# PKBeam/Lanczos-HLS

Hardware: AMD Instinct MI355X
Metric: output Mpixels/s (higher is better)
Workload: dtype f32; 1 GPU; 1920x1080->3840x2160 RGB8 2x Lanczos-3; batch_sets_cycled=3, pattern=gradient, parity_mode=lsb1, kernel=fast, parallelism=32 frames per GPU per step over 1 GPU(s), no data-path collective

## Files before the change

### lanczos-hls_amd/csrc/lanczos_api.hip

```cpp
#include <hip/hip_runtime.h>

#include <algorithm>
#include <cstdio>
#include <cstdlib>
#include <cstring>
#include <map>
#include <mutex>
#include <new>
#include <vector>

#include "../../include/lanczos_hip.h"
#include "lanczos_env.hpp"
#include "lanczos_fast.hpp"
#include "lanczos_layout.hpp"
#include "lanczos_march.hpp"
#include "lanczos_generic.hpp"
#include "lanczos_hls.hpp"
#include "lanczos_rational.hpp"
#include "lanczos_resize.hpp"
#include "lanczos_kernels_common.hpp"
#include "lanczos_taps.hpp"

namespace {

struct PlanKey {
    int in_w, in_h, out_w, out_h, channels, bps, sn, sd, a, hls;
    bool operator<(const PlanKey& o) const { return memcmp(this, &o, sizeof(PlanKey)) < 0; }
};

struct Plan {
    PlanKey key;
    std::vector<hipStream_t> streams;
    lz::AxisTaps H, V;
    lz::PrefixInfo prefix;
    lz::TapTables dev{};
    void* dev_block = nullptr;
    void* host_block = nullptr;
    hipEvent_t uploaded = nullptr;
    hipStream_t upload_stream = nullptr;
    bool captured = false;
    lz::FastConsts fast{};
    bool fast_ok = false;
    lz::RatHost rat;
    lz::RatTables rat_dev{};
    lz::RatPHost ratp;
    lz::RatTables ratp_dev{};
    const float* ratp_w_dev = nullptr;
};

}

struct lanczos_ctx {
    int device = 0;
    hipStream_t stream = nullptr;
    std::map<PlanKey, Plan*> plans;
    lz::LruOrder<PlanKey> plan_order;
    lz::RetireList retired_plans;
    std::vector<void*> kept_dev, kept_host;
    std::mutex mu;
    int last_kernel = LANCZOS_KERNEL_NONE;
    int last_tensor_route = 0;
    int last_route = 0;
    int route_launches = 0;
    int route_seen = 0;
    int last_hip = 0;
    int force = LANCZOS_KERNEL_NONE;
    void* stage_in = nullptr;
    void* stage_out = nullptr;
    size_t stage_in_bytes = 0, stage_out_bytes = 0;
    bool timing = false;
    std::vector<hipEvent_t> ev;
    std::vector<char> ev_prefix_first;
    int ev_used = 0;
    int launches = 0;
    double main_ms = 0, prefix_ms = 0;
#ifdef LZ_PROFILE_BITS
    void* stamp_buf = nullptr;
#endif
    lz::WgTabCache wg_tabs;
    hipStream_t copy_in = nullptr, copy_out = nullptr;
    std::vector<hipEvent_t> pipe_ev;
    void* planar_in = nullptr;
    void* planar_out = nullptr;
    size_t planar_in_bytes = 0, planar_out_bytes = 0;
    lz::ResizeState* resize = nullptr;
};
#ifdef LZ_PROFILE_BITS
static constexpr size_t kStampBytes = 16384 * 8 * 6 * 8;
#endif
static constexpr size_t kMaxPlans = 32;
#ifndef LZ_SPLIT_RULE
#define LZ_SPLIT_RULE 1
#endif

namespace {

#define LZ_HIP(ctx, call)                                  \
    do {                                                   \
        hipError_t e_ = (call);                            \
        if (e_ != hipSuccess) {                            \
            (ctx)->last_hip = (int)e_;                     \
            return LANCZOS_ERR_HIP;                        \
        }                                                  \
    } while (0)

void route_begin(lanczos_ctx* ctx) { ctx->last_route = ctx->route_launches = ctx->route_seen = ctx->last_tensor_route = 0; }
void route_launch(lanczos_ctx* ctx, int main_kernel, int prefix_route) {
    if (ctx->route_launches < 0x7fff) ctx->route_launches++;
    ctx->route_seen |= 1 << prefix_route;
    ctx->last_route = main_kernel | prefix_route << 4 | ctx->route_seen << 8 | ctx->route_launches << 16;
}

void free_plan(Plan* p) {
    if (p->dev_block) (void)hipFree(p->dev_block);
    if (p->host_block) (void)hipHostFree(p->host_block);
    if (p->uploaded) (void)hipEventDestroy(p->uploaded);
    delete p;
}

int get_plan(lanczos_ctx* ctx, const lanczos_desc* d, hipStream_t stream, Plan** out) {
    PlanKey key;
    memset(&key, 0, sizeof(key));
    const bool hls = d->mode == LANCZOS_MODE_HLS;
    key = PlanKey{d->in_w, d->in_h, d->out_w, d->out_h, d->channels, d->bytes_per_sample,
                  d->scale_n, d->scale_d, d->a, hls ? 1 + d->reserved[0] : 0};
    auto it = ctx->plans.find(key);
    if (it != ctx->plans.end()) {
        Plan* p = it->second;
        ctx->plan_order.touch(key);
        if (lz::stream_capturing(stream)) {
            if (p->uploaded && hipEventQuery(p->uploaded) != hipSuccess) LZ_HIP(ctx, hipEventSynchronize(p->uploaded));
            p->captured = true;
        } else {
            if (p->uploaded && stream != p->upload_stream && hipEventQuery(p->uploaded) != hipSuccess)
                LZ_HIP(ctx, hipStreamWaitEvent(stream, p->uploaded, 0));
            lz::note_stream(p->streams, stream);
        }
        *out = p;
        return LANCZOS_OK;
    }
    ctx->retired_plans.reap(false);
    if (ctx->plans.size() >= kMaxPlans && !ctx->plan_order.empty()) {
        const PlanKey old = ctx->plan_order.pop_oldest();
        auto io = ctx->plans.find(old);
        if (io != ctx->plans.end()) {
            Plan* q = io->second;
            if (q->captured) {
                ctx->kept_dev.push_back(q->dev_block);
                ctx->kept_host.push_back(q->host_block);
            } else {
                ctx->retired_plans.retire({q->dev_block}, {q->host_block}, q->streams);
            }
            if (q->uploaded) (void)hipEventDestroy(q->uploaded);
            delete q;
            ctx->plans.erase(io);
        }
    }
    Plan* p = new (std::nothrow) Plan();
    if (!p) return LANCZOS_ERR_NOMEM;
    p->key = key;
    if (hls) {
        lz::build_axis_hls(d->in_w, d->out_w, d->scale_n, d->scale_d, d->a, &p->H, d->reserved[0]);
        lz::build_axis_hls(d->in_h, d->out_h, d->scale_n, d->scale_d, d->a, &p->V, d->reserved[0]);
    } else {
        lz::build_axis(d->in_w, d->out_w, d->scale_n, d->scale_d, d->a, &p->H);
        lz::build_axis(d->in_h, d->out_h, d->scale_n, d->scale_d, d->a, &p->V);
        p->prefix = lz::prefix_info(p->V);
    }
    const int taps = 2 * d->a;
    size_t off_hf = 0;
    size_t off_vf = off_hf + (((size_t)d->out_w * 4 + 7) & ~(size_t)7);
    size_t off_hw = off_vf + (((size_t)d->out_h * 4 + 7) & ~(size_t)7);
    size_t off_vw = off_hw + (size_t)d->out_w * taps * 8;
    size_t off_xw = off_vw + (size_t)d->out_h * taps * 8;
    size_t total = off_xw + (size_t)lz::kFastMaxS * lz::kMaxTaps * 8;
    p->fast_ok = !hls && lz::fast_prepare(*d, p->H, p->V, &p->fast);
    if (!hls && d->scale_d != 1) lz::rat_prepare(*d, p->H, p->V, &p->rat);
    size_t off_hwf = 0, off_vwf = 0, off_hint = 0, off_vint = 0;
    if (p->rat.ok) {
        off_hwf = total;
        off_vwf = off_hwf + (size_t)d->out_w * taps * 4;
        off_hint = off_vwf + (size_t)d->out_h * taps * 4;
        off_vint = off_hint + (((size_t)d->out_w + 7) & ~(size_t)7);
        total = off_vint + (((size_t)d->out_h + 7) & ~(size_t)7);
    }
    size_t off_pw = 0;
    if (p->rat.ok && lz::ratp_has(*d)) lz::ratp_prepare(*d, p->H, p->V, p->rat, &p->ratp);
    if (p->ratp.ok) {
        off_pw = total;
        total += sizeof(p->ratp.phase_w);
    }
    hipError_t e = hipHostMalloc(&p->host_block, total, hipHostMallocDefault);
    if (e != hipSuccess) {
        ctx->last_hip = (int)e;
        delete p;
        return LANCZOS_ERR_HIP;
    }
    struct HostView {
        uint8_t* b;
        uint8_t* data() const { return b; }
    } host{(uint8_t*)p->host_block};
    memset(host.data(), 0, total);
    if (p->rat.ok) {
        memcpy(host.data() + off_hwf, p->rat.h_wf.data(), p->rat.h_wf.size() * 4);
        memcpy(host.data() + off_vwf, p->rat.v_wf.data(), p->rat.v_wf.size() * 4);
        memcpy(host.data() + off_hint, p->rat.h_int.data(), p->rat.h_int.size());
        memcpy(host.data() + off_vint, p->rat.v_int.data(), p->rat.v_int.size());
    }
    if (p->ratp.ok) memcpy(host.data() + off_pw, p->ratp.phase_w, sizeof(p->ratp.phase_w));
    if (p->fast_ok) {
        memcpy(host.data() + off_xw, p->fast.wi, lz::kMaxTaps * 8);
        for (int ph = 1; ph < lz::kFastMaxS; ph++)
            memcpy(host.data() + off_xw + (size_t)ph * lz::kMaxTaps * 8, p->fast.wd[ph], lz::kMaxTaps * 8);
    }
    memcpy(host.data() + off_hf, p->H.first.data(), (size_t)d->out_w * 4);
    memcpy(host.data() + off_vf, p->V.first.data(), (size_t)d->out_h * 4);
    memcpy(host.data() + off_hw, p->H.w.data(), (size_t)d->out_w * taps * 8);
    memcpy(host.data() + off_vw, p->V.w.data(), (size_t)d->out_h * taps * 8);
    const bool capturing = lz::stream_capturing(stream);
    hipStream_t up = stream;
    e = hipMalloc(&p->dev_block, total);
    if (e == hipSuccess && capturing) e = ctx->wg_tabs.eager_stream(&up);
    if (e == hipSuccess && !capturing) e = hipEventCreateWithFlags(&p->uploaded, hipEventDisableTiming);
    if (e != hipSuccess) {
        ctx->last_hip = (int)e;
        free_plan(p);
        return LANCZOS_ERR_HIP;
    }
    e = hipMemcpyAsync(p->dev_block, p->host_block, total, hipMemcpyHostToDevice, up);
    if (e == hipSuccess) e = capturing ? hipStreamSynchronize(up) : hipEventRecord(p->uploaded, stream);
    if (e != hipSuccess) {
        ctx->last_hip = (int)e;
        ctx->retired_plans.retire({p->dev_block}, {p->host_block}, {up});
        if (p->uploaded) (void)hipEventDestroy(p->uploaded);
        delete p;
        return LANCZOS_ERR_HIP;
    }
    if (capturing) {
        p->captured = true;
    } else {
        p->upload_stream = stream;
        p->streams.push_back(stream);
    }
    uint8_t* b = (uint8_t*)p->dev_block;
    p->dev.h_first = (const int32_t*)(b + off_hf);
    p->dev.v_first = (const int32_t*)(b + off_vf);
    p->dev.h_w = (const double*)(b + off_hw);
    p->dev.v_w = (const double*)(b + off_vw);
    p->dev.x_w = (const double*)(b + off_xw);
    if (p->rat.ok) {
        p->rat_dev.h_wf = (const float*)(b + off_hwf);
        p->rat_dev.v_wf = (const float*)(b + off_vwf);
        p->rat_dev.h_int = b + off_hint;
        p->rat_dev.v_int = b + off_vint;
        p->rat_dev.bias = p->rat.bias;
        p->rat_dev.vbias_rne = p->rat.vbias_rne;
        p->rat_dev.near2 = p->rat.near2;
        p->rat_dev.vlim = p->rat.vlim;
        p->rat_dev.tight = p->rat.tight;
    }
    if (p->ratp.ok) {
        p->ratp_dev = p->rat_dev;
        p->ratp_dev.bias = p->ratp.bias;
        p->ratp_dev.vbias_rne = p->ratp.vbias_rne;
        p->ratp_dev.near2 = p->ratp.near2;
        p->ratp_w_dev = (const float*)(b + off_pw);
    }
    ctx->plans[key] = p;
    ctx->plan_order.touch(key);
    *out = p;
    return LANCZOS_OK;
}

int whole_or_strip(const lanczos_desc* d, int* row0, int* rows) {
    if (d->out_rows == 0) {
        *row0 = 0;
        *rows = d->out_h;
    } else {
        *row0 = d->out_row0;
        *rows = d->out_rows;
    }
    return LANCZOS_OK;
}

void strip_input_rows(const lz::AxisTaps& V, int a, int in_h, int row0, int rows, const lz::PrefixInfo& pi,
                      int* in_row0, int* in_rows) {
    int lo = V.first[row0];
    int hi = V.first[row0 + rows - 1] + 2 * a - 1;
    if (row0 < pi.K && pi.M2 - 1 > hi) hi = pi.M2 - 1;
    if (lo < 0) lo = 0;
    if (hi > in_h - 1) hi = in_h - 1;
    *in_row0 = lo;
    *in_rows = hi - lo + 1;
}

}

extern "C" {

const char* lanczos_version(void) {
#ifdef LZ_PROFILE_BITS
    return "lanczos-hls_amd 0.1 (gfx950) +profile-bits";
#else
    return "lanczos-hls_amd 0.1 (gfx950)";
#endif
}

const char* lanczos_strerror(int code) {
    switch (code) {
        case LANCZOS_OK: return "ok";
        case LANCZOS_ERR_BAD_ARG: return "bad argument (null pointer, size, channels, a, or out != in*N/D)";
        case LANCZOS_ERR_UNSUPPORTED: return "unsupported configuration (scale < 1, or a strip that cuts the in-place prefix rows)";
        case LANCZOS_ERR_NO_DEVICE: return "no HIP device";
        case LANCZOS_ERR_HIP: return "HIP runtime error";
        case LANCZOS_ERR_NOMEM: return "out of memory";
        case LANCZOS_ERR_RCCL: return "RCCL call failed (lanczos_multi_last_error)";
        default: return "unknown error";
    }
}

int lanczos_desc_init(lanczos_desc* d, int in_w, int in_h, int channels, int bytes_per_sample, int scale_n,
                      int scale_d, int a) {
    if (!d) return LANCZOS_ERR_BAD_ARG;
    memset(d, 0, sizeof(*d));
    if (scale_n <= 0 || scale_d <= 0) return LANCZOS_ERR_BAD_ARG;
    const int g = lz::gcd(scale_n, scale_d);
    d->in_w = in_w;
    d->in_h = in_h;
    d->scale_n = scale_n / g;
    d->scale_d = scale_d / g;
    d->out_w = (int)((long long)in_w * d->scale_n / d->scale_d);
    d->out_h = (int)((long long)in_h * d->scale_n / d->scale_d);
    d->channels = channels;
    d->bytes_per_sample = bytes_per_sample;
    d->a = a;
    d->mode = LANCZOS_MODE_LSB1;
    return lz::validate(d);
}

int lanczos_validate(const lanczos_desc* d) { return lz::validate(d); }

int lanczos_inplace_rows(const lanczos_desc* d) {
    if (lz::validate(d) != LANCZOS_OK) return -1;
    if (d->mode == LANCZOS_MODE_HLS) return 0;
    lz::AxisTaps V;
    lz::build_axis(d->in_h, d->out_h, d->scale_n, d->scale_d, d->a, &V);
    return lz::prefix_info(V).K;
}

int lanczos_strip_input_rows(const lanczos_desc* d, int out_row0, int out_rows, int* in_row0, int* in_rows) {
    int rc = lz::validate(d);
    if (rc != LANCZOS_OK) return rc;
    if (!in_row0 || !in_rows || out_row0 < 0 || out_rows <= 0 || out_row0 + out_rows > d->out_h)
        return LANCZOS_ERR_BAD_ARG;
    lz::AxisTaps V;
    if (d->mode == LANCZOS_MODE_HLS) {
        lz::build_axis_hls(d->in_h, d->out_h, d->scale_n, d->scale_d, d->a, &V, d->reserved[0]);
        strip_input_rows(V, d->a, d->in_h, out_row0, out_rows, lz::PrefixInfo(), in_row0, in_rows);
        return LANCZOS_OK;
    }
    lz::build_axis(d->in_h, d->out_h, d->scale_n, d->scale_d, d->a, &V);
    strip_input_rows(V, d->a, d->in_h, out_row0, out_rows, lz::prefix_info(V), in_row0, in_rows);
    return LANCZOS_OK;
}

size_t lanczos_in_frame_bytes(const lanczos_desc* d) {
    return d ? (size_t)d->in_w * d->in_h * d->channels * d->bytes_per_sample : 0;
}
size_t lanczos_out_frame_bytes(const lanczos_desc* d) {
    return d ? (size_t)d->out_w * d->out_h * d->channels * d->bytes_per_sample : 0;
}

double lanczos_kernel(double x, int a) { return lz::kernel(x, a); }

double lanczos_kernel_idx(int in_idx, int out_idx, int scale_n, int scale_d, int a) {
    const double SCALE = (double)scale_n / scale_d;
    const double x = (double)out_idx / SCALE;
    return lz::kernel(x - in_idx, a);
}

int lanczos_taps_host(const lanczos_desc* d, int axis, int32_t* first, double* weights) {
    int rc = lz::validate(d);
    if (rc != LANCZOS_OK) return rc;
    if (!first || !weights || (axis != 0 && axis != 1)) return LANCZOS_ERR_BAD_ARG;
    lz::AxisTaps t;
    if (d->mode == LANCZOS_MODE_HLS)
        lz::build_axis_hls(axis == 0 ? d->in_w : d->in_h, axis == 0 ? d->out_w : d->out_h, d->scale_n, d->scale_d, d->a, &t, d->reserved[0]);
    else if (axis == 0)
        lz::build_axis(d->in_w, d->out_w, d->scale_n, d->scale_d, d->a, &t);
    else
        lz::build_axis(d->in_h, d->out_h, d->scale_n, d->scale_d, d->a, &t);
    memcpy(first, t.first.data(), t.first.size() * sizeof(int32_t));
    memcpy(weights, t.w.data(), t.w.size() * sizeof(double));
    return LANCZOS_OK;
}

int lanczos_create(lanczos_ctx** out, int device) {
    if (!out) return LANCZOS_ERR_BAD_ARG;
    *out = nullptr;
    int n = 0;
    if (hipGetDeviceCount(&n) != hipSuccess || n <= 0) return LANCZOS_ERR_NO_DEVICE;
    if (device < 0 || device >= n) return LANCZOS_ERR_NO_DEVICE;
    (void)lz::env();
    lanczos_ctx* ctx = new (std::nothrow) lanczos_ctx();
    if (!ctx) return LANCZOS_ERR_NOMEM;
    ctx->device = device;
    if (hipSetDevice(device) != hipSuccess ||
        hipStreamCreateWithFlags(&ctx->stream, hipStreamNonBlocking) != hipSuccess) {
        delete ctx;
        return LANCZOS_ERR_HIP;
    }
    *out = ctx;
    return LANCZOS_OK;
}

#ifdef LZ_PROFILE_BITS
static void diag_report(lanczos_ctx* ctx, FILE* out) {
    if (!ctx->stamp_buf) return;
    {
        std::vector<unsigned long long> h(kStampBytes / 8);
        if (hipMemcpy(h.data(), ctx->stamp_buf, kStampBytes, hipMemcpyDeviceToHost) == hipSuccess) {
            double sum[5] = {0, 0, 0, 0, 0}, ticks = 0;
            long n = 0;
            for (size_t i = 0; i + 5 < (size_t)16384 * 8 * 3; i += 6)
                if (h[i + 5]) {
                    for (int k = 0; k < 5; k++) sum[k] += (double)h[i + k];
                    ticks += (double)h[i + 5];
                    n++;
                }
            {
                std::map<unsigned long long, std::vector<std::pair<unsigned long long, int>>> ev;
                const size_t off = (size_t)16384 * 8 * 3;
                long wgs = 0;
                unsigned long long tmin = ~0ull, tmax = 0;
                for (size_t i = off; i + 2 < h.size(); i += 3) {
                    if (!h[i + 1]) continue;
                    const unsigned hw = (unsigned)h[i + 2];
                    const unsigned long long key = ((h[i + 2] >> 32) << 16) | (((hw >> 13) & 7) << 8) | (((hw >> 12) & 1) << 4) | ((hw >> 8) & 15);
                    ev[key].push_back({h[i], +1});
                    ev[key].push_back({h[i + 1], -1});
                    if (h[i] < tmin) tmin = h[i];
                    if (h[i + 1] > tmax) tmax = h[i + 1];
                    wgs++;
                }
                double avg = 0;
                int peak = 0;
                for (auto& kv : ev) {
                    std::sort(kv.second.begin(), kv.second.end());
                    int cur = 0;
                    unsigned long long last = tmin, area = 0;
                    for (auto& e : kv.second) {
                        area += (unsigned long long)cur * (e.first - last);
                        last = e.first;
                        cur += e.second;
                        if (cur > peak) peak = cur;
                    }
                    avg += (double)area / (double)(tmax - tmin ? tmax - tmin : 1);
                }
                {
                    std::vector<double> st, life;
                    for (size_t i = off; i + 2 < h.size(); i += 3)
                        if (h[i + 1]) {
                            st.push_back((h[i] - tmin) / 100.0);
                            life.push_back((h[i + 1] - h[i]) / 100.0);
                        }
                    std::sort(st.begin(), st.end());
                    std::sort(life.begin(), life.end());
                    if (!st.empty())
                        fprintf(out, "CENSUS start us: p50=%.1f p90=%.1f max=%.1f | lifetime us: min=%.1f p10=%.1f p50=%.1f p90=%.1f max=%.1f\n",
                                st[st.size() / 2], st[st.size() * 9 / 10], st.back(), life.front(), life[life.size() / 10],
                                life[life.size() / 2], life[life.size() * 9 / 10], life.back());
                }
                if (!lz::env().census_dump.empty()) {
                    FILE* df = fopen(lz::env().census_dump.c_str(), "w");
                    if (df) {
                        for (size_t i = off, k = 0; i + 2 < h.size(); i += 3, k++)
                            if (h[i + 1])
                                fprintf(df, "%zu %llu %llu %u %u\n", k, h[i] - tmin, h[i + 1] - tmin, (unsigned)(h[i + 2] >> 32),
                                        (unsigned)h[i + 2]);
                        fclose(df);
                    }
                }
                if (wgs)
                    fprintf(out, "CENSUS wgs=%ld distinct_cus=%zu span=%.1f us avg_resident_wgs_per_cu=%.2f peak=%d\n", wgs,
                            ev.size(), (tmax - tmin) / 100.0, avg / ev.size(), peak);
            }
            if (n)
                fprintf(out, "STAMP waves=%ld ticks/wave=%.1f cycles/tick: issue=%.0f hpass=%.0f commit=%.0f vpass=%.0f barrier=%.0f\n",
                        n, ticks / n, sum[0] / ticks, sum[1] / ticks, sum[2] / ticks, sum[3] / ticks, sum[4] / ticks);
            for (int w = 0; w < 6; w++) {
                double s6[5] = {0, 0, 0, 0, 0}, tk = 0;
                for (size_t i = (size_t)w * 6; i + 5 < (size_t)16384 * 8 * 3; i += 36)
                    if (h[i + 5]) {
                        for (int k = 0; k < 5; k++) s6[k] += (double)h[i + k];
                        tk += (double)h[i + 5];
                    }
                if (tk > 0)
                    fprintf(out, "STAMP wave %d: issue=%.0f hpass=%.0f commit=%.0f vpass=%.0f barrier=%.0f\n", w, s6[0] / tk, s6[1] / tk,
                            s6[2] / tk, s6[3] / tk, s6[4] / tk);
            }
        }
    }
}
#endif

int lanczos_destroy(lanczos_ctx* ctx) {
    if (!ctx) return LANCZOS_ERR_BAD_ARG;
    (void)hipSetDevice(ctx->device);
    (void)hipDeviceSynchronize();
    ctx->retired_plans.reap(true);
    ctx->wg_tabs.release_all();
    for (auto& kv : ctx->plans) free_plan(kv.second);
    ctx->plans.clear();
    for (void* p : ctx->kept_dev) (void)hipFree(p);
    for (void* p : ctx->kept_host) (void)hipHostFree(p);
    delete ctx->resize;
#ifdef LZ_PROFILE_BITS
    if (ctx->stamp_buf) {
        diag_report(ctx, stderr);
        (void)hipFree(ctx->stamp_buf);
    }
#endif
    for (hipEvent_t e : ctx->ev) (void)hipEventDestroy(e);
    for (hipEvent_t e : ctx->pipe_ev) (void)hipEventDestroy(e);
    if (ctx->copy_in) (void)hipStreamDestroy(ctx->copy_in);
    if (ctx->copy_out) (void)hipStreamDestroy(ctx->copy_out);
    if (ctx->planar_in) (void)hipFree(ctx->planar_in);
    if (ctx->planar_out) (void)hipFree(ctx->planar_out);
    if (ctx->stage_in) (void)hipFree(ctx->stage_in);
    if (ctx->stage_out) (void)hipFree(ctx->stage_out);
    if (ctx->stream) (void)hipStreamDestroy(ctx->stream);
    delete ctx;
    return LANCZOS_OK;
}

int lanczos_timing_enable(lanczos_ctx* ctx, int on) {
    if (!ctx) return LANCZOS_ERR_BAD_ARG;
    ctx->timing = on != 0;
    return LANCZOS_OK;
}

static int timing_flush(lanczos_ctx* ctx) {
    const int used = ctx->ev_used;
    ctx->ev_used = 0;
    for (int i = 0; i + 2 < used; i += 3) {
        float a = 0, b = 0;
        LZ_HIP(ctx, hipEventSynchronize(ctx->ev[i + 2]));
        LZ_HIP(ctx, hipEventElapsedTime(&a, ctx->ev[i], ctx->ev[i + 1]));
        LZ_HIP(ctx, hipEventElapsedTime(&b, ctx->ev[i + 1], ctx->ev[i + 2]));
        const bool prefix_first = ctx->ev_prefix_first[i / 3] != 0;
        ctx->main_ms += prefix_first ? b : a;
        ctx->prefix_ms += prefix_first ? a : b;
        ctx->launches++;
    }
    return LANCZOS_OK;
}

int lanczos_timing_read(lanczos_ctx* ctx, int* launches, double* main_kernel_ms, double* prefix_kernel_ms) {
    if (!ctx) return LANCZOS_ERR_BAD_ARG;
    std::lock_guard<std::mutex> lock(ctx->mu);
    (void)hipSetDevice(ctx->device);
    int rc = timing_flush(ctx);
    if (rc != LANCZOS_OK) return rc;
    if (launches) *launches = ctx->launches;
    if (main_kernel_ms) *main_kernel_ms = ctx->main_ms;
    if (prefix_kernel_ms) *prefix_kernel_ms = ctx->prefix_ms;
    ctx->launches = 0;
    ctx->main_ms = ctx->prefix_ms = 0;
    return LANCZOS_OK;
}

int lanczos_last_kernel(const lanczos_ctx* ctx) { return ctx ? ctx->last_kernel : LANCZOS_KERNEL_NONE; }
int lanczos_last_route(const lanczos_ctx* ctx) { return ctx ? ctx->last_route : 0; }
int lanczos_last_hip_error(const lanczos_ctx* ctx) { return ctx ? ctx->last_hip : 0; }

int lanczos_force_kernel(lanczos_ctx* ctx, int family) {
    if (!ctx || family < LANCZOS_KERNEL_NONE || family > LANCZOS_KERNEL_FAST) return LANCZOS_ERR_BAD_ARG;
    ctx->force = family;
    return LANCZOS_OK;
}

static hipError_t launch_prefix_front(const lanczos_desc* d, const lz::FrameGeom& g, const Plan* p, hipStream_t stream) {
#define LZ_PREFIX_REG_CONFIGS(X)                                                                                        \
    X(uint8_t, 2, 2) X(uint8_t, 2, 3) X(uint8_t, 2, 4) X(uint8_t, 3, 2) X(uint8_t, 3, 3) X(uint8_t, 3, 4) X(uint8_t, 4, 2) \
    X(uint8_t, 4, 3) X(uint8_t, 4, 4) X(uint16_t, 2, 3) X(uint16_t, 2, 4) X(uint16_t, 3, 3) X(uint16_t, 3, 4)
    bool have = false;
#define X(T, S, A)                                                                                                    \
    if (d->bytes_per_sample == (int)sizeof(T) && d->scale_n == S && d->a == A && p->prefix.K == lz::prefix_K(S, A) && \
        p->prefix.M == lz::prefix_M(S, A) && p->prefix.M2 == lz::prefix_M2(S, A))                                    \
        have = true;
    LZ_PREFIX_REG_CONFIGS(X)
#undef X
    if (!have) return hipErrorNotSupported;
    const int samples_w = d->out_w * d->channels;
    dim3 grid((samples_w + 127) / 128, g.frames);
#define X(T, S, A)                                                                                  \
    if (d->bytes_per_sample == (int)sizeof(T) && d->scale_n == S && d->a == A)                      \
        hipLaunchKernelGGL((lz::k_prefix_reg<T, S, A>), grid, dim3(128), 0, stream, g, p->dev);
    LZ_PREFIX_REG_CONFIGS(X)
#undef X
    return hipGetLastError();
}

static int resample_device_locked(lanczos_ctx* ctx, const lanczos_desc* d, const void* d_in, void* d_out, int frames,
                                  size_t in_frame_stride, size_t out_frame_stride, void* stream_v, bool in_split = false) {
    int rc;
    LZ_HIP(ctx, hipSetDevice(ctx->device));
    hipStream_t stream = (hipStream_t)stream_v;
    Plan* p = nullptr;
    rc = get_plan(ctx, d, stream, &p);
    if (rc != LANCZOS_OK) return rc;

    int row0, rows;
    whole_or_strip(d, &row0, &rows);
    int in_row0, in_rows;
    strip_input_rows(p->V, d->a, d->in_h, row0, rows, p->prefix, &in_row0, &in_rows);
    const bool has_prefix = row0 < p->prefix.K;
    if (has_prefix) {
        if (row0 != 0) return LANCZOS_ERR_UNSUPPORTED;
    }

    lz::FrameGeom g{};
    g.in = (const uint8_t*)d_in;
    g.out = (uint8_t*)d_out;
    g.in_pitch = d->in_w * d->channels * d->bytes_per_sample;
    g.out_pitch = d->out_w * d->channels * d->bytes_per_sample;
    g.in_frame_stride = in_frame_stride ? in_frame_stride : (size_t)g.in_pitch * in_rows;
    g.out_frame_stride = out_frame_stride ? out_frame_stride : (size_t)g.out_pitch * rows;
    g.in_w = d->in_w;
    g.in_h = d->in_h;
    g.out_w = d->out_w;
    g.out_h = d->out_h;
    g.channels = d->channels;
    g.a = d->a;
    g.in_row0 = in_row0;
    g.in_rows = in_rows;
    g.out_row0 = row0;
    g.out_rows = rows;
    g.skip_rows = has_prefix ? p->prefix.K : 0;
    g.frames = frames;
    g.hls_bp = d->mode == LANCZOS_MODE_HLS ? d->reserved[0] : 0;
    g.debug_skip = 0;
    g.stamps = nullptr;
#ifdef LZ_PROFILE_BITS
    g.debug_skip = lz::env().debug_skip;
    if (lz::env().stamp) {
        if (!ctx->stamp_buf) (void)hipMalloc(&ctx->stamp_buf, kStampBytes), (void)hipMemset(ctx->stamp_buf, 0, kStampBytes);
        g.stamps = (unsigned long long*)ctx->stamp_buf;
    }
#endif
    if (d->mode == LANCZOS_MODE_HLS) {
        if (ctx->force == LANCZOS_KERNEL_FAST || ctx->force == LANCZOS_KERNEL_GENERIC) return LANCZOS_ERR_UNSUPPORTED;
        if (d->channels > 4 || 2 * d->a > 2 * lz::kMaxA) return LANCZOS_ERR_UNSUPPORTED;
        if (frames > 65535) return LANCZOS_ERR_UNSUPPORTED;
    }
    bool prefix_fused = false;
    bool use_fast = p->fast_ok && ctx->force != LANCZOS_KERNEL_GENERIC &&
                    lz::fast_supports(*d, g);
    const bool use_rat = !use_fast && p->rat.ok && ctx->force != LANCZOS_KERNEL_GENERIC && lz::rat_supports(*d, g);
    if (ctx->force == LANCZOS_KERNEL_FAST && !use_fast && !use_rat) return LANCZOS_ERR_UNSUPPORTED;

    hipEvent_t ev0 = nullptr, ev1 = nullptr, ev2 = nullptr;
    if (ctx->timing) {
        if (ctx->ev_used + 3 > 3 * 4096) {
            rc = timing_flush(ctx);
            if (rc != LANCZOS_OK) return rc;
        }
        while ((int)ctx->ev.size() < ctx->ev_used + 3) {
            hipEvent_t e;
            LZ_HIP(ctx, hipEventCreate(&e));
            ctx->ev.push_back(e);
        }
        ctx->ev_prefix_first.resize(ctx->ev.size() / 3 + 1, 0);
        ev0 = ctx->ev[ctx->ev_used];
        ev1 = ctx->ev[ctx->ev_used + 1];
        ev2 = ctx->ev[ctx->ev_used + 2];
        LZ_HIP(ctx, hipEventRecord(ev0, stream));
    }
    if (d->mode == LANCZOS_MODE_HLS) {
        const int tiles_x = (d->out_w + lz::kHlsTileW - 1) / lz::kHlsTileW;
        const int tiles_y = (rows + lz::kHlsTileH - 1) / lz::kHlsTileH;
        dim3 grid(tiles_x * tiles_y, frames);
        if (d->bytes_per_sample == 1)
            hipLaunchKernelGGL(lz::k_hls<uint8_t>, grid, dim3(lz::kHlsThreads), 0, stream, g, p->dev);
        else
            hipLaunchKernelGGL(lz::k_hls<uint16_t>, grid, dim3(lz::kHlsThreads), 0, stream, g, p->dev);
        LZ_HIP(ctx, hipGetLastError());
        ctx->last_kernel = LANCZOS_KERNEL_HLS;
        route_launch(ctx, LANCZOS_ROUTE_MAIN_HLS, LANCZOS_ROUTE_PREFIX_NONE);
        if (ev0) {
            LZ_HIP(ctx, hipEventRecord(ev1, stream));
            LZ_HIP(ctx, hipEventRecord(ev2, stream));
            ctx->ev_prefix_first[ctx->ev_used / 3] = 0;
            ctx->ev_used += 3;
        }
        return LANCZOS_OK;
    }
    bool prefix_front = false;
    int route_main = LANCZOS_ROUTE_MAIN_NONE;
    if (use_fast) {
        hipError_t e;
        if (lz::env().tile_kernel || !lz::march_supports(g)) {
            e = lz::fast_launch(*d, g, p->dev, p->fast, stream);
            route_main = LANCZOS_ROUTE_MAIN_TILE;
        } else {
            lz::FrameGeom gm = g;
            if (!in_split) {
                bool dummy = false;
                e = lz::march_launch(*d, gm, p->dev, p->fast, stream, &dummy, &ctx->wg_tabs, true);
                const int pf = ctx->wg_tabs.pref_frames;
                const bool split = frames >= 2 * pf || (LZ_SPLIT_RULE && ctx->wg_tabs.wg_per_cu >= 4 && frames >= pf + pf / 2);
                if (e == hipSuccess && pf >= 8 && split) {
                    for (int f0 = 0; f0 < frames; f0 += pf) {
                        const int nf = frames - f0 < pf ? frames - f0 : pf;
                        rc = resample_device_locked(ctx, d, (const uint8_t*)d_in + (size_t)f0 * g.in_frame_stride,
                                                    (uint8_t*)d_out + (size_t)f0 * g.out_frame_stride, nf, g.in_frame_stride,
                                                    g.out_frame_stride, stream_v, true);
                        if (rc != LANCZOS_OK) return rc;
                    }
                    return LANCZOS_OK;
                }
            }
            if (has_prefix) {
                gm.prefix_K = p->prefix.K;
                gm.prefix_M = p->prefix.M;
                gm.prefix_M2 = p->prefix.M2;
                e = lz::march_launch(*d, gm, p->dev, p->fast, stream, &prefix_fused, &ctx->wg_tabs, true);
                if (e == hipSuccess && !prefix_fused) {
                    gm.prefix_K = gm.prefix_M = gm.prefix_M2 = 0;
                    if (!lz::env().separate_prefix && d->scale_d == 1 && d->in_h >= p->prefix.M2) {
                        hipError_t pe = launch_prefix_front(d, g, p, stream);
                        if (pe == hipSuccess) {
                            prefix_front = true;
                            if (ev1) LZ_HIP(ctx, hipEventRecord(ev1, stream));
                        } else if (pe != hipErrorNotSupported) e = pe;
                    }
                }
            } else {
                e = hipSuccess;
            }
            if (e == hipSuccess) e = lz::march_launch(*d, gm, p->dev, p->fast, stream, &prefix_fused, &ctx->wg_tabs);
            route_main = row0 + rows <= g.skip_rows ? LANCZOS_ROUTE_MAIN_NONE : LANCZOS_ROUTE_MAIN_MARCH;
        }
        if (e != hipSuccess) {
            ctx->last_hip = (int)e;
            return LANCZOS_ERR_HIP;
        }
        ctx->last_kernel = LANCZOS_KERNEL_FAST;
    } else if (use_rat && p->ratp.ok && !lz::env().no_ratp) {
        hipError_t e = lz::ratp_launch(*d, g, p->dev, p->ratp_dev, p->ratp_w_dev, stream);
        if (e != hipSuccess) {
            ctx->last_hip = (int)e;
            return LANCZOS_ERR_HIP;
        }
        ctx->last_kernel = LANCZOS_KERNEL_FAST;
        route_main = LANCZOS_ROUTE_MAIN_RATP;
    } else if (use_rat) {
        const int row_bytes = d->out_w * d->channels * d->bytes_per_sample;
        const int tiles_x = (row_bytes + lz::kRatTileRowBytes - 1) / lz::kRatTileRowBytes;
        const int tiles_y = (rows + lz::kRatTileH - 1) / lz::kRatTileH;
        dim3 grid(tiles_x * tiles_y, frames);
        const bool ex = d->mode == LANCZOS_MODE_EXACT;
#define LZ_RAT(T, TAPS)                                                                                                  \
    do {                                                                                                                 \
        if (ex) hipLaunchKernelGGL((lz::k_rat<T, TAPS, true>), grid, dim3(lz::kRatThreads), 0, stream, g, p->dev, p->rat_dev);  \
        else hipLaunchKernelGGL((lz::k_rat<T, TAPS, false>), grid, dim3(lz::kRatThreads), 0, stream, g, p->dev, p->rat_dev);    \
    } while (0)
        if (d->bytes_per_sample == 1) {
            if (d->a == 2) LZ_RAT(uint8_t, 4);
            else if (d->a == 3) LZ_RAT(uint8_t, 6);
            else LZ_RAT(uint8_t, 8);
        } else {
            if (d->a == 2) LZ_RAT(uint16_t, 4);
            else if (d->a == 3) LZ_RAT(uint16_t, 6);
            else LZ_RAT(uint16_t, 8);
        }
#undef LZ_RAT
        LZ_HIP(ctx, hipGetLastError());
        ctx->last_kernel = LANCZOS_KERNEL_FAST;
        route_main = LANCZOS_ROUTE_MAIN_RAT;
    } else {
        const int samples_w = d->out_w * d->channels;
        const int tiles_x = (samples_w + lz::kGenTileW - 1) / lz::kGenTileW;
        const int tiles_y = (rows + lz::kGenTileH - 1) / lz::kGenTileH;
        dim3 grid(tiles_x * tiles_y, frames);
        if (d->bytes_per_sample == 1)
            hipLaunchKernelGGL(lz::k_generic<uint8_t>, grid, dim3(lz::kGenTileW), 0, stream, g, p->dev);
        else
            hipLaunchKernelGGL(lz::k_generic<uint16_t>, grid, dim3(lz::kGenTileW), 0, stream, g, p->dev);
        LZ_HIP(ctx, hipGetLastError());
        ctx->last_kernel = LANCZOS_KERNEL_GENERIC;
        route_main = LANCZOS_ROUTE_MAIN_GENERIC;
    }
    int route_prefix = prefix_fused ? LANCZOS_ROUTE_PREFIX_RIDING : (prefix_front ? LANCZOS_ROUTE_PREFIX_FRONT : LANCZOS_ROUTE_PREFIX_NONE);
    if (ev1 && !prefix_front) LZ_HIP(ctx, hipEventRecord(ev1, stream));

    if (has_prefix && !prefix_fused && !prefix_front) {
        const int samples_w = d->out_w * d->channels;
        int bw = 128;
        while (bw > 32 && (size_t)(p->prefix.M + p->prefix.M2) * bw * d->bytes_per_sample > 60 * 1024) bw >>= 1;
        const bool streamed = (size_t)(p->prefix.M + p->prefix.M2) * bw * d->bytes_per_sample > 60 * 1024;
        if (streamed) bw = 128;
        dim3 grid((samples_w + bw - 1) / bw, frames);
#define LZ_PREFIX_STREAM(T, TAPS) \
    hipLaunchKernelGGL((lz::k_prefix_stream<T, TAPS>), grid, dim3(128), 0, stream, g, p->dev, p->prefix.K, p->prefix.M)
        route_prefix = streamed ? LANCZOS_ROUTE_PREFIX_STREAMED : LANCZOS_ROUTE_PREFIX_BEHIND;
        if (streamed) {
            if (d->bytes_per_sample == 1) {
                if (d->a == 2) LZ_PREFIX_STREAM(uint8_t, 4);
                else if (d->a == 3) LZ_PREFIX_STREAM(uint8_t, 6);
                else LZ_PREFIX_STREAM(uint8_t, 8);
            } else {
                if (d->a == 2) LZ_PREFIX_STREAM(uint16_t, 4);
                else if (d->a == 3) LZ_PREFIX_STREAM(uint16_t, 6);
                else LZ_PREFIX_STREAM(uint16_t, 8);
            }
        } else
#define LZ_PREFIX(T, TAPS)                                                                                       \
    hipLaunchKernelGGL((lz::k_prefix<T, TAPS>), grid, dim3(bw), (size_t)(p->prefix.M + p->prefix.M2) * bw * sizeof(T), stream, g, \
                       p->dev, p->prefix.K, p->prefix.M, p->prefix.M2)
        if (d->bytes_per_sample == 1) {
            if (d->a == 2) LZ_PREFIX(uint8_t, 4);
            else if (d->a == 3) LZ_PREFIX(uint8_t, 6);
            else LZ_PREFIX(uint8_t, 8);
        } else {
            if (d->a == 2) LZ_PREFIX(uint16_t, 4);
            else if (d->a == 3) LZ_PREFIX(uint16_t, 6);
            else LZ_PREFIX(uint16_t, 8);
        }
#undef LZ_PREFIX
#undef LZ_PREFIX_STREAM
        LZ_HIP(ctx, hipGetLastError());
    }
    route_launch(ctx, route_main, route_prefix);
    if (ev2) {
        LZ_HIP(ctx, hipEventRecord(ev2, stream));
        ctx->ev_prefix_first[ctx->ev_used / 3] = prefix_front ? 1 : 0;
        ctx->ev_used += 3;
    }
    return LANCZOS_OK;
}

int lanczos_resample_device(lanczos_ctx* ctx, const lanczos_desc* d, const void* d_in, void* d_out, int frames,
                            size_t in_frame_stride, size_t out_frame_stride, void* stream_v) {
    if (!ctx || !d_in || !d_out || frames <= 0) return LANCZOS_ERR_BAD_ARG;
    int rc = lz::validate(d);
    if (rc != LANCZOS_OK) return rc;
    std::lock_guard<std::mutex> lock(ctx->mu);
    route_begin(ctx);
    return resample_device_locked(ctx, d, d_in, d_out, frames, in_frame_stride, out_frame_stride, stream_v);
}

int lanczos_host_alloc(void** p, size_t bytes) {
    if (!p || bytes == 0) return LANCZOS_ERR_BAD_ARG;
    *p = nullptr;
    return hipHostMalloc(p, bytes, hipHostMallocDefault) == hipSuccess ? LANCZOS_OK : LANCZOS_ERR_NOMEM;
}

int lanczos_host_free(void* p) {
    if (!p) return LANCZOS_OK;
    return hipHostFree(p) == hipSuccess ? LANCZOS_OK : LANCZOS_ERR_HIP;
}

int lanczos_resample_host(lanczos_ctx* ctx, const lanczos_desc* d, const void* in, void* out, int frames) {
    if (!ctx || !in || !out || frames <= 0) return LANCZOS_ERR_BAD_ARG;
    int rc = lz::validate(d);
    if (rc != LANCZOS_OK) return rc;
    std::lock_guard<std::mutex> lock(ctx->mu);
    LZ_HIP(ctx, hipSetDevice(ctx->device));
    if (!ctx->stream) return LANCZOS_ERR_HIP;
    route_begin(ctx);
    Plan* p = nullptr;
    rc = get_plan(ctx, d, ctx->stream, &p);
    if (rc != LANCZOS_OK) return rc;
    int row0, rows, in_row0, in_rows;
    whole_or_strip(d, &row0, &rows);
    strip_input_rows(p->V, d->a, d->in_h, row0, rows, p->prefix, &in_row0, &in_rows);
    const size_t in_frame = (size_t)d->in_w * d->channels * d->bytes_per_sample * in_rows;
    const size_t out_frame = (size_t)d->out_w * d->channels * d->bytes_per_sample * rows;
    const size_t in_bytes = in_frame * frames, out_bytes = out_frame * frames;
    if (ctx->stage_in_bytes < in_bytes) {
        if (ctx->stage_in) (void)hipFree(ctx->stage_in);
        ctx->stage_in = nullptr;
        ctx->stage_in_bytes = 0;
        LZ_HIP(ctx, hipMalloc(&ctx->stage_in, in_bytes));
        ctx->stage_in_bytes = in_bytes;
    }
    if (ctx->stage_out_bytes < out_bytes) {
        if (ctx->stage_out) (void)hipFree(ctx->stage_out);
        ctx->stage_out = nullptr;
        ctx->stage_out_bytes = 0;
        LZ_HIP(ctx, hipMalloc(&ctx->stage_out, out_bytes));
        ctx->stage_out_bytes = out_bytes;
    }
    if (!ctx->copy_in) LZ_HIP(ctx, hipStreamCreateWithFlags(&ctx->copy_in, hipStreamNonBlocking));
    if (!ctx->copy_out) LZ_HIP(ctx, hipStreamCreateWithFlags(&ctx->copy_out, hipStreamNonBlocking));
    int group = frames >= 8 ? 4 : (frames >= 2 ? (frames + 1) / 2 : 1);
    if ((frames + group - 1) / group > 64) group = (frames + 63) / 64;
    const int ngroups = (frames + group - 1) / group;
    while ((int)ctx->pipe_ev.size() < 2 * ngroups) {
        hipEvent_t e;
        LZ_HIP(ctx, hipEventCreateWithFlags(&e, hipEventDisableTiming));
        ctx->pipe_ev.push_back(e);
// ... 331 lines not shown
```

### lanczos-hls_amd/csrc/lanczos_generic.hpp

```cpp
#pragma once
#include "lanczos_kernels_common.hpp"
#include "lanczos_taps.hpp"

namespace lz {

constexpr int kGenTileW = 256;
constexpr int kGenTileH = 32;
constexpr int kGenMaxHRows = kGenTileH + 2 * kMaxA;

template <typename T>
__global__ __launch_bounds__(kGenTileW) void k_generic(FrameGeom g, TapTables t) {
    __shared__ T hbuf[kGenMaxHRows][kGenTileW];

    const int taps = 2 * g.a;
    const int C = g.channels;
    const int samples_w = g.out_w * C;
    const int tiles_x = (samples_w + kGenTileW - 1) / kGenTileW;
    const int tx = blockIdx.x % tiles_x;
    const int ty = blockIdx.x / tiles_x;
    const int frame = blockIdx.y;

    const int y_begin = g.out_row0 + ty * kGenTileH;
    int y_end = y_begin + kGenTileH;
    if (y_end > g.out_row0 + g.out_rows) y_end = g.out_row0 + g.out_rows;
    if (y_end <= g.skip_rows) return;

    int r_lo = t.v_first[y_begin];
    int r_hi = t.v_first[y_end - 1] + taps - 1;
    if (r_lo < 0) r_lo = 0;
    if (r_hi > g.in_h - 1) r_hi = g.in_h - 1;

    const int j = tx * kGenTileW + threadIdx.x;
    const bool active = j < samples_w;
    const uint8_t* in_f = g.in + (size_t)frame * g.in_frame_stride;
    uint8_t* out_f = g.out + (size_t)frame * g.out_frame_stride;

    if (active) {
        const int xx = j / C, c = j - xx * C;
        const int first = t.h_first[xx];
        double w[kMaxTaps];
        int idx[kMaxTaps];
#pragma unroll
        for (int k = 0; k < kMaxTaps; k++) {
            if (k < taps) {
                w[k] = t.h_w[(size_t)xx * taps + k];
                int i = first + k;
                i = i < 0 ? 0 : (i > g.in_w - 1 ? g.in_w - 1 : i);
                idx[k] = i * C + c;
            } else {
                w[k] = 0.0;
                idx[k] = 0;
            }
        }
        for (int r = r_lo; r <= r_hi; r++) {
            const T* row = (const T*)(in_f + (size_t)(r - g.in_row0) * g.in_pitch);
            double sum = 0;
#pragma unroll
            for (int k = 0; k < kMaxTaps; k++)
                if (k < taps) sum += (double)row[idx[k]] * w[k];
            hbuf[r - r_lo][threadIdx.x] = store_convert<T>(sum);
        }
    }
    __syncthreads();

    if (active) {
        for (int y = y_begin; y < y_end; y++) {
            if (y < g.skip_rows) continue;
            const int first = t.v_first[y];
            const double* wv = t.v_w + (size_t)y * taps;
            double sum = 0;
            for (int k = 0; k < taps; k++) {
                int i = first + k;
                i = i < r_lo ? r_lo : (i > r_hi ? r_hi : i);
                sum += (double)hbuf[i - r_lo][threadIdx.x] * wv[k];
            }
            T* orow = (T*)(out_f + (size_t)(y - g.out_row0) * g.out_pitch);
            orow[j] = store_convert<T>(sum);
        }
    }
}

template <typename T, int TAPS>
__global__ __launch_bounds__(128) void k_prefix(FrameGeom g, TapTables t, int K, int M, int M2) {
    const int C = g.channels;
    const int samples_w = g.out_w * C;
    const int j = blockIdx.x * blockDim.x + threadIdx.x;
    const int frame = blockIdx.y;
    if (j >= samples_w) return;
    const uint8_t* in_f = g.in + (size_t)frame * g.in_frame_stride;
    uint8_t* out_f = g.out + (size_t)frame * g.out_frame_stride;

    extern __shared__ __attribute__((aligned(16))) uint8_t prefix_smem[];
    const int bw = blockDim.x;
    T* hs = (T*)prefix_smem;
    T* os = hs + (size_t)M2 * bw;
    const int tl = threadIdx.x;

    {
        const int xx = j / C, c = j - xx * C;
        const int first = t.h_first[xx];
        int idx[TAPS];
        double w[TAPS];
#pragma unroll
        for (int k = 0; k < TAPS; k++) {
            int i = first + k;
            i = i < 0 ? 0 : (i > g.in_w - 1 ? g.in_w - 1 : i);
            idx[k] = i * C + c;
            w[k] = t.h_w[(size_t)xx * TAPS + k];
        }
#pragma unroll 4
        for (int r = 0; r < M2; r++) {
            const T* row = (const T*)(in_f + (size_t)(r - g.in_row0) * g.in_pitch);
            T v[TAPS];
#pragma unroll
            for (int k = 0; k < TAPS; k++) v[k] = row[idx[k]];
            double sum = 0;
#pragma unroll
            for (int k = 0; k < TAPS; k++) sum += (double)v[k] * w[k];
            hs[r * bw + tl] = store_convert<T>(sum);
        }
    }
    for (int xx = M - 1; xx >= 0; xx--) {
        const int first = t.v_first[xx];
        const double* wv = t.v_w + (size_t)xx * TAPS;
        double sum = 0;
#pragma unroll
        for (int k = 0; k < TAPS; k++) {
            int i = first + k;
            i = i < 0 ? 0 : (i > g.in_h - 1 ? g.in_h - 1 : i);
            const T v = i > xx ? os[i * bw + tl] : hs[i * bw + tl];
            sum += (double)v * wv[k];
        }
        os[xx * bw + tl] = store_convert<T>(sum);
    }
    for (int xx = 0; xx < K; xx++) {
        if (xx < g.out_row0 || xx >= g.out_row0 + g.out_rows) continue;
        T* orow = (T*)(out_f + (size_t)(xx - g.out_row0) * g.out_pitch);
        orow[j] = os[xx * bw + tl];
    }
}

template <typename T, int TAPS>
__global__ __launch_bounds__(128) void k_prefix_stream(FrameGeom g, TapTables t, int K, int M) {
    constexpr int HR = 16, OR = 8, CH = 8;
    static_assert(TAPS <= 8 && CH + TAPS - 1 <= HR && TAPS / 2 + 1 <= OR, "ring sizes");
    const int C = g.channels;
    const int samples_w = g.out_w * C;
    const int j = blockIdx.x * blockDim.x + threadIdx.x;
    const int frame = blockIdx.y;
    if (j >= samples_w) return;
    const uint8_t* in_f = g.in + (size_t)frame * g.in_frame_stride;
    uint8_t* out_f = g.out + (size_t)frame * g.out_frame_stride;
    __shared__ T hs[HR][128];
    __shared__ T os[OR][128];
    const int tl = threadIdx.x;
    const int xx_h = j / C, c = j - xx_h * C;
    int idx[TAPS];
    double w[TAPS];
    {
        const int first = t.h_first[xx_h];
#pragma unroll
        for (int k = 0; k < TAPS; k++) {
            int i = first + k;
            i = i < 0 ? 0 : (i > g.in_w - 1 ? g.in_w - 1 : i);
            idx[k] = i * C + c;
            w[k] = t.h_w[(size_t)xx_h * TAPS + k];
        }
    }
    auto vfirst = [&](int xx) { return t.v_first[xx]; };
    int h_lo = vfirst(M - 1) + TAPS;
    if (h_lo > g.in_h) h_lo = g.in_h;
    for (int xx = M - 1; xx >= 0; xx--) {
        const int first = vfirst(xx);
        const int need = first < 0 ? 0 : first;
        while (h_lo > need) {
            const int r0 = h_lo - CH < 0 ? 0 : h_lo - CH;
            T v[CH][TAPS];
#pragma unroll
            for (int rr = 0; rr < CH; rr++) {
                const int r = r0 + rr < h_lo ? r0 + rr : h_lo - 1;
                const T* row = (const T*)(in_f + (size_t)(r - g.in_row0) * g.in_pitch);
#pragma unroll
                for (int k = 0; k < TAPS; k++) v[rr][k] = row[idx[k]];
            }
#pragma unroll
            for (int rr = 0; rr < CH; rr++) {
                if (r0 + rr >= h_lo) break;
                double sum = 0;
#pragma unroll
                for (int k = 0; k < TAPS; k++) sum += (double)v[rr][k] * w[k];
                hs[(r0 + rr) & (HR - 1)][tl] = store_convert<T>(sum);
            }
            h_lo = r0;
        }
        const double* wv = t.v_w + (size_t)xx * TAPS;
        double sum = 0;
#pragma unroll
        for (int k = 0; k < TAPS; k++) {
            int i = first + k;
            i = i < 0 ? 0 : (i > g.in_h - 1 ? g.in_h - 1 : i);
            const T v = i > xx ? os[i & (OR - 1)][tl] : hs[i & (HR - 1)][tl];
            sum += (double)v * wv[k];
        }
        const T o = store_convert<T>(sum);
        os[xx & (OR - 1)][tl] = o;
        if (xx < K && xx >= g.out_row0 && xx < g.out_row0 + g.out_rows)
            ((T*)(out_f + (size_t)(xx - g.out_row0) * g.out_pitch))[j] = o;
    }
}

constexpr int prefix_last_tap(int o, int S, int A) { return o / S + A; }
constexpr int prefix_K(int S, int A) {
    int k = 0;
    for (int o = 0; o < 4 * A * S + 8; o++)
        if (prefix_last_tap(o, S, A) > o) k = o + 1;
    return k;
}
constexpr int prefix_M(int S, int A) {
    int m = prefix_K(S, A);
    for (int o = 0; o < prefix_K(S, A); o++)
        if (prefix_last_tap(o, S, A) + 1 > m) m = prefix_last_tap(o, S, A) + 1;
    return m;
}
constexpr int prefix_M2(int S, int A) {
    int m2 = 0;
    for (int o = 0; o < prefix_M(S, A); o++)
        if (prefix_last_tap(o, S, A) + 1 > m2) m2 = prefix_last_tap(o, S, A) + 1;
    return m2;
}

template <typename T, int S, int A>
__global__ __launch_bounds__(128) void k_prefix_reg(FrameGeom g, TapTables t) {
    constexpr int TAPS = 2 * A, K = prefix_K(S, A), M = prefix_M(S, A), M2 = prefix_M2(S, A);
    const int C = g.channels;
    const int samples_w = g.out_w * C;
    const int j = blockIdx.x * blockDim.x + threadIdx.x;
    const int frame = blockIdx.y;
    if (j >= samples_w) return;
    const uint8_t* in_f = g.in + (size_t)frame * g.in_frame_stride;
    uint8_t* out_f = g.out + (size_t)frame * g.out_frame_stride;
    T hs[M2], os[M];
    {
        const int xx = j / C, c = j - xx * C;
        const int first = t.h_first[xx];
        int idx[TAPS];
        double w[TAPS];
#pragma unroll
        for (int k = 0; k < TAPS; k++) {
            int i = first + k;
            i = i < 0 ? 0 : (i > g.in_w - 1 ? g.in_w - 1 : i);
            idx[k] = i * C + c;
            w[k] = t.h_w[(size_t)xx * TAPS + k];
        }
#pragma unroll
        for (int r = 0; r < M2; r++) {
            const T* row = (const T*)(in_f + (size_t)r * g.in_pitch);
            T v[TAPS];
#pragma unroll
            for (int k = 0; k < TAPS; k++) v[k] = row[idx[k]];
            double sum = 0;
#pragma unroll
            for (int k = 0; k < TAPS; k++) sum += (double)v[k] * w[k];
            hs[r] = store_convert<T>(sum);
        }
    }
#pragma unroll
    for (int xx = M - 1; xx >= 0; xx--) {
        constexpr int dummy = 0;
        (void)dummy;
        const int first = xx / S - A + 1;
        const double* wv = t.v_w + (size_t)xx * TAPS;
        double sum = 0;
#pragma unroll
        for (int k = 0; k < TAPS; k++) {
            const int i = first + k < 0 ? 0 : first + k;
            const T v = i > xx ? os[i < M ? i : M - 1] : hs[i < M2 ? i : M2 - 1];
            sum += (double)v * wv[k];
        }
        os[xx] = store_convert<T>(sum);
    }
#pragma unroll
    for (int xx = 0; xx < K; xx++) {
        if (xx < g.out_row0 || xx >= g.out_row0 + g.out_rows) continue;
        T* orow = (T*)(out_f + (size_t)(xx - g.out_row0) * g.out_pitch);
        orow[j] = os[xx];
    }
}

}
```

### lanczos-hls_amd/csrc/lanczos_kernels_common.hpp

```cpp
#pragma once
#include <hip/hip_runtime.h>

#include <cstdint>

#ifndef LZ_STORE_AUX
#define LZ_STORE_AUX 18
#endif

namespace lz {

struct WgEntry {
    int frame, tx, m_b, m_e;
};

struct FrameGeom {
    const uint8_t* in;
    uint8_t* out;
    unsigned long long in_frame_stride, out_frame_stride;
    int in_pitch, out_pitch;
    int in_w, in_h, out_w, out_h;
    int channels, a;
    int in_row0, in_rows;
    int out_row0, out_rows;
    int skip_rows;
    int frames;
    unsigned long long* stamps;
    int n_main, wg_per_frame, prefix_blocks_per_frame, prefix_K, prefix_M, prefix_M2;
    int hls_bp;
    int debug_skip;
    const WgEntry* wg_tab;
    int wg_segs;
};

struct TapTables {
    const int32_t* h_first;
    const double* h_w;
    const int32_t* v_first;
    const double* v_w;
    const double* x_w;
};

template <typename T>
__device__ __forceinline__ T store_convert(double x) {
    constexpr double kMax = sizeof(T) == 1 ? 255.0 : 65535.0;
    if (x > kMax) return (T)kMax;
    if (x < 0) return (T)0;
    return (T)(unsigned)x;
}

}
```

Before: 1.278 million Mpix/s.

## Vectorize prefix-row kernel to process packed dword output columns per thread

Rewrites the top-of-frame prefix kernel so each thread produces one 32-bit word of output, covering several packed samples, instead of one byte sample. Input is read as dwords and unpacked with shifts and funnel-style windowing for non-dword-aligned channel counts such as RGB. The aim is fewer, wider memory transactions and fewer threads in this edge kernel. It adds heavier per-thread register and ALU work, and a byte-path fallback for misaligned or non-integer tap layouts. The prefix covers only a few output rows, so its share of total frame time is likely small.

```diff
diff --git a/lanczos-hls_amd/csrc/lanczos_api.hip b/lanczos-hls_amd/csrc/lanczos_api.hip
--- a/lanczos-hls_amd/csrc/lanczos_api.hip
+++ b/lanczos-hls_amd/csrc/lanczos_api.hip
@@ -33,6 +33,7 @@
     std::vector<hipStream_t> streams;
     lz::AxisTaps H, V;
     lz::PrefixInfo prefix;
+    bool h_first_integer = false;
     lz::TapTables dev{};
     void* dev_block = nullptr;
     void* host_block = nullptr;
@@ -166,6 +167,9 @@
         lz::build_axis(d->in_w, d->out_w, d->scale_n, d->scale_d, d->a, &p->H);
         lz::build_axis(d->in_h, d->out_h, d->scale_n, d->scale_d, d->a, &p->V);
         p->prefix = lz::prefix_info(p->V);
+        p->h_first_integer = d->scale_d == 1;
+        for (int xx = 0; xx < d->out_w && p->h_first_integer; xx++)
+            p->h_first_integer = p->H.first[xx] == xx / d->scale_n - d->a + 1;
     }
     const int taps = 2 * d->a;
     size_t off_hf = 0;
@@ -591,14 +595,28 @@
         have = true;
     LZ_PREFIX_REG_CONFIGS(X)
 #undef X
-    if (!have) return hipErrorNotSupported;
+    if (!have || !p->h_first_integer) return hipErrorNotSupported;
     const int samples_w = d->out_w * d->channels;
-    dim3 grid((samples_w + 127) / 128, g.frames);
+    const size_t row_bytes = (size_t)samples_w * d->bytes_per_sample;
+    const bool dwords = lz::prefix_dword_channels(d->channels) && row_bytes % 4 == 0 &&
+                        ((uintptr_t)g.in | (uintptr_t)g.out | (uintptr_t)g.in_pitch | (uintptr_t)g.out_pitch |
+                         (uintptr_t)g.in_frame_stride | (uintptr_t)g.out_frame_stride) % 4 == 0;
+    if (dwords) {
+        const int row_dw = (int)(row_bytes / 4);
+        dim3 grid((row_dw + lz::kPrefixRegBlock - 1) / lz::kPrefixRegBlock, g.frames);
 #define X(T, S, A)                                                                                  \
     if (d->bytes_per_sample == (int)sizeof(T) && d->scale_n == S && d->a == A)                      \
-        hipLaunchKernelGGL((lz::k_prefix_reg<T, S, A>), grid, dim3(128), 0, stream, g, p->dev);
-    LZ_PREFIX_REG_CONFIGS(X)
+        hipLaunchKernelGGL((lz::k_prefix_reg<T, S, A>), grid, dim3(lz::kPrefixRegBlock), 0, stream, g, p->dev);
+        LZ_PREFIX_REG_CONFIGS(X)
 #undef X
+    } else {
+        dim3 grid((samples_w + 127) / 128, g.frames);
+#define X(T, S, A)                                                                                  \
+    if (d->bytes_per_sample == (int)sizeof(T) && d->scale_n == S && d->a == A)                      \
+        hipLaunchKernelGGL((lz::k_prefix_reg_bytes<T, S, A>), grid, dim3(128), 0, stream, g, p->dev);
+        LZ_PREFIX_REG_CONFIGS(X)
+#undef X
+    }
     return hipGetLastError();
 }
 
diff --git a/lanczos-hls_amd/csrc/lanczos_generic.hpp b/lanczos-hls_amd/csrc/lanczos_generic.hpp
--- a/lanczos-hls_amd/csrc/lanczos_generic.hpp
+++ b/lanczos-hls_amd/csrc/lanczos_generic.hpp
@@ -230,7 +230,7 @@
 }
 
 template <typename T, int S, int A>
-__global__ __launch_bounds__(128) void k_prefix_reg(FrameGeom g, TapTables t) {
+__global__ __launch_bounds__(128) void k_prefix_reg_bytes(FrameGeom g, TapTables t) {
     constexpr int TAPS = 2 * A, K = prefix_K(S, A), M = prefix_M(S, A), M2 = prefix_M2(S, A);
     const int C = g.channels;
     const int samples_w = g.out_w * C;
@@ -266,8 +266,6 @@
     }
 #pragma unroll
     for (int xx = M - 1; xx >= 0; xx--) {
-        constexpr int dummy = 0;
-        (void)dummy;
         const int first = xx / S - A + 1;
         const double* wv = t.v_w + (size_t)xx * TAPS;
         double sum = 0;
@@ -287,4 +285,170 @@
     }
 }
 
-}
+template <typename T, int S, int A, int C>
+struct PrefixDword {
+    static constexpr int SB = (int)sizeof(T), NS = 4 / SB, TAPS = 2 * A;
+    static constexpr int K = prefix_K(S, A), M = prefix_M(S, A), M2 = prefix_M2(S, A);
+    static constexpr bool kStrided = (C * SB) % 4 == 0;
+    static constexpr int WN = ((TAPS - 1) * C * SB + SB + 3) / 4;
+    static constexpr int tap0_byte(int j) { return ((j / C / S - A + 1) * C + j % C) * SB; }
+    static constexpr int q_max() {
+        int q = 0;
+        for (int d = A * S * C; d < A * S * C + 12 * C * S; d++) {
+            int lo = tap0_byte(NS * d);
+            for (int e = 1; e < NS; e++) lo = tap0_byte(NS * d + e) < lo ? tap0_byte(NS * d + e) : lo;
+            for (int e = 0; e < NS; e++) {
+                const int qe = (tap0_byte(NS * d + e) - (lo & ~3)) >> 2;
+                q = qe > q ? qe : q;
+            }
+        }
+        return q;
+    }
+    static constexpr int QMAX = q_max(), ND = WN + 1 + QMAX;
+};
+
+template <typename T, int S, int A, int C>
+__host__ __device__ inline void prefix_dword_column(const uint8_t* in_f, int in_pitch, int in_w, const double* h_w, const double* v_w,
+                                                    int d, uint32_t* out) {
+    using P = PrefixDword<T, S, A, C>;
+    constexpr int SB = P::SB, NS = P::NS, TAPS = P::TAPS, K = P::K, M = P::M, M2 = P::M2;
+    constexpr uint32_t MASK = SB == 1 ? 0xffu : 0xffffu;
+    const int j0 = d * NS;
+    uint32_t hsp[M2];
+    if constexpr (P::kStrided) {
+        const int xx = j0 / C, cd = (j0 - xx * C) * SB / 4;
+        const int first = xx / S - A + 1;
+        int idx[TAPS];
+        double w[TAPS];
+#pragma unroll
+        for (int k = 0; k < TAPS; k++) {
+            int i = first + k;
+            i = i < 0 ? 0 : (i > in_w - 1 ? in_w - 1 : i);
+            idx[k] = i * (C * SB / 4) + cd;
+            w[k] = h_w[(size_t)xx * TAPS + k];
+        }
+#pragma unroll
+        for (int r = 0; r < M2; r++) {
+            const uint32_t* row = (const uint32_t*)(in_f + (size_t)r * in_pitch);
+            uint32_t v[TAPS];
+#pragma unroll
+            for (int k = 0; k < TAPS; k++) v[k] = row[idx[k]];
+            uint32_t pk = 0;
+#pragma unroll
+            for (int e = 0; e < NS; e++) {
+                double sum = 0;
+#pragma unroll
+                for (int k = 0; k < TAPS; k++) sum += (double)((v[k] >> (8 * SB * e)) & MASK) * w[k];
+                pk |= (uint32_t)store_convert<T>(sum) << (8 * SB * e);
+            }
+            hsp[r] = pk;
+        }
+    } else {
+        constexpr int WN = P::WN, QMAX = P::QMAX, ND = P::ND;
+        const int row_dw = in_pitch >> 2;
+        int q[NS], m8[NS], lo = 0;
+        double w[NS][TAPS];
+#pragma unroll
+        for (int e = 0; e < NS; e++) {
+            const int j = j0 + e, xx = j / C, c = j - xx * C;
+            q[e] = ((xx / S - A + 1) * C + c) * SB;
+            lo = e == 0 || q[e] < lo ? q[e] : lo;
+#pragma unroll
+            for (int k = 0; k < TAPS; k++) w[e][k] = h_w[(size_t)xx * TAPS + k];
+        }
+        const int base = lo >> 2;
+        int di[ND];
+#pragma unroll
+        for (int i = 0; i < ND; i++) {
+            const int x = base + i;
+            di[i] = x < 0 ? 0 : (x > row_dw - 1 ? row_dw - 1 : x);
+        }
+#pragma unroll
+        for (int e = 0; e < NS; e++) {
+            const int rel = q[e] - base * 4;
+            q[e] = rel >> 2;
+            m8[e] = (rel & 3) * 8;
+        }
+#pragma unroll
+        for (int r = 0; r < M2; r++) {
+            const uint32_t* row = (const uint32_t*)(in_f + (size_t)r * in_pitch);
+            uint32_t raw[ND];
+#pragma unroll
+            for (int i = 0; i < ND; i++) raw[i] = row[di[i]];
+            uint32_t pk = 0;
+#pragma unroll
+            for (int e = 0; e < NS; e++) {
+                uint32_t sh[WN + 1], win[WN];
+#pragma unroll
+                for (int i = 0; i <= WN; i++) {
+                    sh[i] = raw[i];
+#pragma unroll
+                    for (int qq = 1; qq <= QMAX; qq++) sh[i] = q[e] == qq ? raw[i + qq] : sh[i];
+                }
+#pragma unroll
+                for (int i = 0; i < WN; i++) win[i] = (uint32_t)((((uint64_t)sh[i + 1] << 32) | sh[i]) >> m8[e]);
+                double sum = 0;
+#pragma unroll
+                for (int k = 0; k < TAPS; k++)
+                    sum += (double)((win[(k * C * SB) >> 2] >> (8 * ((k * C * SB) & 3))) & MASK) * w[e][k];
+                pk |= (uint32_t)store_convert<T>(sum) << (8 * SB * e);
+            }
+            hsp[r] = pk;
+        }
+    }
+#pragma unroll
+    for (int xx = 0; xx < K; xx++) out[xx] = 0;
+#pragma unroll
+    for (int e = 0; e < NS; e++) {
+        T os[M];
+#pragma unroll
+        for (int xx = M - 1; xx >= 0; xx--) {
+            const int first = xx / S - A + 1;
+            const double* wv = v_w + (size_t)xx * TAPS;
+            double sum = 0;
+#pragma unroll
+            for (int k = 0; k < TAPS; k++) {
+                const int i = first + k < 0 ? 0 : first + k;
+                const T v = i > xx ? os[i < M ? i : M - 1] : (T)((hsp[i < M2 ? i : M2 - 1] >> (8 * SB * e)) & MASK);
+                sum += (double)v * wv[k];
+            }
+            os[xx] = store_convert<T>(sum);
+            if (xx < K) out[xx] |= (uint32_t)os[xx] << (8 * SB * e);
+        }
+    }
+}
+
+template <int K>
+__host__ __device__ inline void prefix_dword_store(uint8_t* out_f, int out_pitch, int out_row0, int out_rows, int d, const uint32_t* o) {
+#pragma unroll
+    for (int xx = 0; xx < K; xx++) {
+        if (xx < out_row0 || xx >= out_row0 + out_rows) continue;
+        uint32_t* orow = (uint32_t*)(out_f + (size_t)(xx - out_row0) * out_pitch);
+        orow[d] = o[xx];
+    }
+}
+
+#ifndef LZ_PREFIX_BLOCK
+#define LZ_PREFIX_BLOCK 128
+#endif
+constexpr int kPrefixRegBlock = LZ_PREFIX_BLOCK;
+
+inline bool prefix_dword_channels(int c) { return c == 1 || c == 3 || c == 4; }
+
+template <typename T, int S, int A>
+__global__ __launch_bounds__(kPrefixRegBlock) void k_prefix_reg(FrameGeom g, TapTables t) {
+    constexpr int K = prefix_K(S, A);
+    const int row_dw = (g.out_w * g.channels * (int)sizeof(T)) >> 2;
+    const int d = blockIdx.x * kPrefixRegBlock + threadIdx.x;
+    const int frame = blockIdx.y;
+    if (d >= row_dw) return;
+    const uint8_t* in_f = g.in + (size_t)frame * g.in_frame_stride;
+    uint8_t* out_f = g.out + (size_t)frame * g.out_frame_stride;
+    uint32_t o[K];
+    if (g.channels == 3) prefix_dword_column<T, S, A, 3>(in_f, g.in_pitch, g.in_w, t.h_w, t.v_w, d, o);
+    else if (g.channels == 4) prefix_dword_column<T, S, A, 4>(in_f, g.in_pitch, g.in_w, t.h_w, t.v_w, d, o);
+    else prefix_dword_column<T, S, A, 1>(in_f, g.in_pitch, g.in_w, t.h_w, t.v_w, d, o);
+    prefix_dword_store<K>(out_f, g.out_pitch, g.out_row0, g.out_rows, d, o);
+}
+
+}
diff --git a/lanczos-hls_amd/csrc/lanczos_kernels_common.hpp b/lanczos-hls_amd/csrc/lanczos_kernels_common.hpp
--- a/lanczos-hls_amd/csrc/lanczos_kernels_common.hpp
+++ b/lanczos-hls_amd/csrc/lanczos_kernels_common.hpp
@@ -41,7 +41,7 @@
 };
 
 template <typename T>
-__device__ __forceinline__ T store_convert(double x) {
+__host__ __device__ __forceinline__ T store_convert(double x) {
     constexpr double kMax = sizeof(T) == 1 ? 255.0 : 65535.0;
     if (x > kMax) return (T)kMax;
     if (x < 0) return (T)0;
```

New measurement: 1.229 million Mpix/s. 0.962x the previous value.
